# cokwa/bitHTM

Measured on AMD Instinct MI355X. Metric: HTM timesteps/sec (SP + TM, learning on), 65536 cols x 32 cells, higher is better.
Workload: dtype u32 bit-packed / f64 + f32 permanences; 1 GPU; configs[2]: 65536 columns x 32 cells, SP + TM learning on, 1 MI355X; input_dim=1024, column_dim=65536, cell_dim=32, active_columns=1311, patterns=50, pretrain_steps=500, segments=96476, segment_slots=128, hip_graph=True, hip_graph_requested=True, pipelined=True, repetitions=15, streamed_calls=True

## Files before the change

bithtm_amd/_lib.py:

```python

import ctypes as C
import os

HERE = os.path.dirname(os.path.abspath(__file__))
LIB_PATH = os.path.join(HERE, "libbithtm_hip.so")
ABI_VERSION = 4


class HtmConfig(C.Structure):
    _fields_ = [
        ("struct_bytes", C.c_uint32), ("device", C.c_int32),
        ("input_dim", C.c_int32), ("column_dim", C.c_int32), ("cell_dim", C.c_int32),
        ("active_columns", C.c_int32), ("enable_sp", C.c_int32), ("enable_tm", C.c_int32),
        ("sp_permanence_threshold", C.c_double), ("sp_delta_on", C.c_double), ("sp_delta_off", C.c_double),
        ("boost_coefficient", C.c_float), ("duty_momentum", C.c_float), ("duty_increment", C.c_float),
        ("tm_learn_active", C.c_double), ("tm_learn_inactive", C.c_double),
        ("tm_punish_active", C.c_double), ("tm_punish_inactive", C.c_double),
        ("tm_learn_prune", C.c_int32), ("tm_punish_prune", C.c_int32),
        ("tm_permanence_initial", C.c_float), ("tm_permanence_threshold", C.c_float),
        ("segment_activation_threshold", C.c_int32), ("segment_matching_threshold", C.c_int32),
        ("segment_sampling_synapses", C.c_int32),
        ("segment_capacity", C.c_int32), ("segment_capacity_local", C.c_int32), ("segment_slots", C.c_int32),
        ("seed", C.c_uint32), ("shard_rank", C.c_int32), ("shard_world", C.c_int32), ("use_caller_stream", C.c_int32),
        ("stream", C.c_void_p),
    ]


class HtmInfo(C.Structure):
    _fields_ = [
        ("step_index", C.c_int64), ("segments", C.c_int32), ("local_segments", C.c_int32), ("matching_segments", C.c_int32),
        ("winner_cells", C.c_int32), ("active_cells", C.c_int32), ("has_distal_state", C.c_int32),
        ("has_winner_cells", C.c_int32), ("capacity_error", C.c_int32), ("words_per_row", C.c_int32),
        ("new_segment_requests", C.c_int32), ("recycled_segments", C.c_int32), ("appended_segments", C.c_int32),
        ("work_items", C.c_int32), ("select_fallbacks", C.c_int32), ("candidate_exact_steps", C.c_int32), ("hot_select_steps", C.c_int32),
        ("select_zoom_steps", C.c_int32),
    ]


class HtmStepRecord(C.Structure):
    _fields_ = [(name, C.c_int32) for name in (
        "active_columns", "bursting_columns", "predicted_columns_before", "predicted_columns", "active_cells", "winner_cells",
        "segments", "new_segments")]


class HtmRunRecord(C.Structure):
    _fields_ = [("struct_bytes", C.c_uint32), ("records", C.c_void_p), ("active_column", C.c_void_p), ("column_prediction", C.c_void_p)]


F_ACTIVE_COLUMN, F_OVERLAPS, F_BOOSTED, F_DUTY_CYCLE, F_CELL_ACTIVATION, F_CELL_PREDICTION = 1, 2, 3, 4, 5, 6
F_WINNER_WORDS, F_BURSTING, F_WINNER_CELL, F_SEG_CELL, F_SEG_NSYN, F_SEG_PRESYN, F_SEG_PERM = 7, 8, 9, 10, 11, 12, 13
F_SEGCOUNT, F_SEG_POTENTIAL, F_MATCH_SEGMENT, F_MATCH_INFO, F_MATCH_JITTER, F_CELL_MAX_JITTER = 14, 15, 16, 17, 18, 19
F_SEG_GID = 20
PLAN_GRAPH, PLAN_PIPELINED, PLAN_LEAN, PLAN_SCAN_LARGE = 1, 2, 4, 8
SP_OVERLAP, SP_BOOST, SP_SELECT, SP_ACTIVE, SP_LEARN, SP_DUTY, SP_COMMIT = 1, 2, 3, 4, 5, 6, 7

EXPORTS = {
    "htm_abi_version": (C.c_int, []),
    "htm_create": (C.c_int, [C.POINTER(HtmConfig), C.POINTER(C.c_void_p)]),
    "htm_destroy": (None, [C.c_void_p]),
    "htm_last_error": (C.c_char_p, [C.c_void_p]),
    "htm_sp_set_permanence": (C.c_int, [C.c_void_p, C.c_void_p, C.c_int32, C.c_int32]),
    "htm_set_epsilon": (C.c_int, [C.c_void_p, C.c_float]),
    "htm_sp_get_permanence": (C.c_int, [C.c_void_p, C.c_void_p, C.c_int32, C.c_int32]),
    "htm_step": (C.c_int, [C.c_void_p, C.c_void_p, C.c_int32]),
    "htm_sp_step": (C.c_int, [C.c_void_p, C.c_void_p, C.c_int32]),
    "htm_sp_phase": (C.c_int, [C.c_void_p, C.c_int32, C.c_void_p, C.c_int64]),
    "htm_tm_step": (C.c_int, [C.c_void_p, C.c_void_p, C.c_int32, C.c_int32, C.c_int32]),
    "htm_tm_update": (C.c_int, [C.c_void_p, C.c_void_p, C.c_void_p, C.c_void_p, C.c_int32, C.c_void_p]),
    "htm_tm_scan": (C.c_int, [C.c_void_p, C.c_void_p]),
    "htm_run": (C.c_int, [C.c_void_p, C.c_void_p, C.c_int32, C.c_int32, C.c_int32, C.c_int32]),
    "htm_prepare": (C.c_int, [C.c_void_p, C.c_void_p, C.c_int32, C.c_int32, C.c_int32, C.c_int32]),
    "htm_run_recorded": (C.c_int, [C.c_void_p, C.c_void_p, C.c_int32, C.c_int32, C.c_int32, C.c_int32, C.POINTER(HtmRunRecord)]),
    "htm_prepare_recorded": (C.c_int, [C.c_void_p, C.c_void_p, C.c_int32, C.c_int32, C.c_int32, C.c_int32]),
    "htm_reset": (C.c_int, [C.c_void_p]),
    "htm_set_run_resets": (C.c_int, [C.c_void_p, C.c_void_p, C.c_int32]),
    "htm_predicted_input": (C.c_int, [C.c_void_p, C.c_void_p]),
    "htm_set_run_predicted_input": (C.c_int, [C.c_void_p, C.c_void_p]),
    "htm_graph_count": (C.c_int, [C.c_void_p]),
    "htm_run_plan": (C.c_int, [C.c_void_p, C.c_int32, C.c_int32]),
    "htm_bank_upload": (C.c_int, [C.c_void_p, C.c_void_p, C.c_int32, C.POINTER(C.c_void_p)]),
    "htm_shard_record_bytes": (C.c_int64, [C.c_void_p]),
    "htm_shard_begin": (C.c_int, [C.c_void_p, C.c_void_p, C.c_int32, C.c_void_p, C.c_int32, C.c_void_p]),
    "htm_shard_finish": (C.c_int, [C.c_void_p, C.c_void_p, C.c_int32]),
    "htm_shard_unique_id": (C.c_int, [C.c_void_p]),
    "htm_shard_comm_init": (C.c_int, [C.c_void_p, C.c_void_p]),
    "htm_shard_step": (C.c_int, [C.c_void_p, C.c_void_p, C.c_int32, C.c_void_p, C.c_int32]),
    "htm_shard_comm_size": (C.c_int, [C.c_void_p]),
    "htm_shard_graph_ok": (C.c_int, [C.c_void_p]),
    "htm_shard_run": (C.c_int, [C.c_void_p, C.c_void_p, C.c_int32, C.c_int32, C.c_int32, C.c_int32]),
    "htm_shard_group_run": (C.c_int, [C.POINTER(C.c_void_p), C.c_int32, C.POINTER(C.c_void_p), C.c_int32, C.c_int32, C.c_int32, C.c_int32]),
    "htm_rccl_selftest": (C.c_int, [C.c_int32]),
    "htm_keyed_draws": (C.c_int, [C.c_uint32, C.c_int32, C.c_uint32, C.c_void_p, C.c_void_p, C.c_int64, C.c_void_p]),
    "htm_shard_group_step": (C.c_int, [C.POINTER(C.c_void_p), C.c_int32, C.POINTER(C.c_void_p), C.c_int32, C.c_void_p, C.c_int32]),
    "htm_populate": (C.c_int, [C.c_void_p, C.c_int64, C.c_int64, C.c_int32, C.c_int32, C.c_double, C.c_double, C.c_uint32]),
    "htm_sync": (C.c_int, [C.c_void_p]),
    "htm_get_stream": (C.c_int, [C.c_void_p, C.POINTER(C.c_void_p)]),
    "htm_get_info": (C.c_int, [C.c_void_p, C.POINTER(HtmInfo)]),
    "htm_read": (C.c_int64, [C.c_void_p, C.c_int32, C.c_void_p, C.c_int64]),
    "htm_read_rows": (C.c_int64, [C.c_void_p, C.c_int32, C.c_int64, C.c_int64, C.c_void_p, C.c_int64]),
    "htm_import_begin": (C.c_int, [C.c_void_p, C.c_int64]),
    "htm_write": (C.c_int, [C.c_void_p, C.c_int32, C.c_void_p, C.c_int64]),
    "htm_import_commit": (C.c_int, [C.c_void_p, C.c_int32, C.c_int32, C.c_int32, C.c_int32, C.c_int32]),
    "htm_profile": (C.c_int, [C.c_void_p, C.c_int32]),
    "htm_profile_read": (C.c_int, [C.c_void_p, C.c_int32, C.POINTER(C.c_char_p), C.POINTER(C.c_double),
                                   C.POINTER(C.c_int64)]),
# ... 47 lines not shown
```

bithtm_amd/csrc/htm_dev.h:

```cpp
#ifndef BITHTM_HTM_DEV_H
#define BITHTM_HTM_DEV_H

typedef unsigned long long u64;

#define SEL_MAX_PASSES 6
#define SEL_DIGIT 12
#define SEL_BINS 4096
#define HIST_REP 4
#define SEL_COARSE 64
#define COARSE_REP 16
#define COARSE_STRIDE 1024
#define FAN_COUNTERS 16
#define FAN_STRIDE 32
#define HIST0_FINE (HIST_REP * SEL_BINS)
#define HIST0_PAR (HIST0_FINE + COARSE_REP * COARSE_STRIDE)
#define RB 512
#define SCAN_SEGS 64
#define DEAD_CAP 256
#define SHARD_HOT_KEYS 4
#define CAND_CAP 256
#define WIN_LDS 4096
#define MAX_SLOTS 512
#define SYN_CONNECTED 0x80000000u
#define SYN_CELL 0x7FFFFFFF
// ... 24 lines not shown

__host__ __device__ __forceinline__ int sel_shift(int pass) { return pass < 5 ? 52 - SEL_DIGIT * pass : 0; }
__host__ __device__ __forceinline__ int sel_bits(int pass) { return pass < 5 ? SEL_DIGIT : 4; }

struct Counters {
    uint32_t step[2];
    int32_t S;
    int32_t n_win[2];
    int32_t has_winner[2];
    int32_t has_distal;
    uint32_t cm_dense_step;
    int32_t n_active_cells;
    alignas(128) int32_t n_work[2];
    int32_t n_bind[2];
    alignas(128) int32_t n_work_last;
    int32_t sel_fallbacks;
    int32_t cand_exact;
    int32_t hot_selects;
    int32_t sel_zooms;
    uint32_t emit_epoch;
    int32_t n_un;
    int32_t n_recycled, n_new, S_old;
    int32_t L;
    int32_t n_lfree;
    int32_t error;
    u64 sel_prefix[2];
    uint32_t sel_krem[2];
    uint32_t sel_win[2];
    uint32_t sel_win_global;
    u64 sel_pass_prefix[2][SEL_MAX_PASSES + 1];
    uint32_t sel_pass_krem[2][SEL_MAX_PASSES + 1];
};

struct Dev {
    int I, W, W4, Ipad, C, K, k, E, Scap, work_cap, sel_passes, colwords, low_zero, cand_d, cand_pairwise, cand_others, cand_speculate, cand_take_all, cand_zoom, poll_delay;
    int win_offset;
    int cls_rows_max;
    int LK, KP, WPC;
    int world, c0, c1;
    int sel_lo, sel_hi, sel_k;
    int Lcap, n_cand;
    int hot_budget, hot_target;
    int cand_cap;
    double sp_thr, sp_don, sp_doff;
    float coef, mom, dinc;
    double lrn_act, lrn_inact, pun_act, pun_inact;
    int lrn_prune, pun_prune;
    float perm_init, perm_thr;
    float eps;
    int act_thr, match_thr, sample;
    uint32_t seed;
    double *perm;
    uint32_t *mask;
    float *duty;
    int *overlap[2];
    double *boosted[2];
    u64 *key[2];
    uint32_t *hist;
    uint32_t *hist0;
    uint32_t *sel_blk;
    uint32_t *sel_rec;
    int *active_cols[2];
    uint32_t *input_stage;
    uint32_t *act[2];
    uint32_t *pred[2];
    uint32_t *win[2];
    uint32_t *colbits[2];
    int *winners[2];
    uint8_t *bursting;
    int *actw_id;
    uint32_t *winw_idx;
    uint8_t *actcnt;
    uint32_t *act_list;
    uint16_t *col_rank[2];
    uint32_t *unacc_word;
    uint32_t *fan;
    int *unacc_list;
    int *seg_cell;
    int *seg_nsyn;
    int *presyn;
    float *sperm;
    int *segcount;
    uint32_t *cellmax[2];
    uint32_t *match_bits[2];
    uint32_t *seg_info;
    float *seg_jit;
    uint32_t *work;
    int *recyc_cnt;
    int *recyc_cnt2;
    int *recyc_need;
    int *seg_gid;
    int *g2l;
    uint32_t *dead_bits;
    int *lfree;
    int *asg_gid;
    int *cand_cols;
    int *dead_list;
    const uint32_t *punish;
    unsigned char *send;
    Counters *ctr;
    unsigned long long *trace;
    uint32_t trace_until;
};

__device__ __forceinline__ int lane_id() { return threadIdx.x & 63; }
__device__ __forceinline__ u64 lanemask_lt() { return (1ull << lane_id()) - 1ull; }
// ... 156 lines not shown
```

bithtm_amd/csrc/htm_engine.hip:

```cpp

#include <hip/hip_runtime.h>
#include <hip/hip_ext.h>
#include <dlfcn.h>
#include <stdint.h>
#include <stdio.h>
#include <string.h>
#include <algorithm>
#include <climits>
#include <chrono>
#include <map>
#include <mutex>
#include <string>
#include <tuple>
#include <type_traits>
#include <vector>

#include "../../include/bithtm_hip.h"
#include "htm_fexp.h"
#include "htm_rng.h"

#include "htm_dev.h"
#include "htm_sp_kernels.h"
#include "htm_tm_kernels.h"
#include "htm_pipeline.h"
// ... 486 lines not shown

extern "C" int htm_abi_version(void) { return BITHTM_ABI_VERSION; }

extern "C" const char *htm_last_error(const htm_handle *h) { return h ? h->err.c_str() : g_create_error.c_str(); }

extern "C" void htm_destroy(htm_handle *h) {
    if (!h) return;
    {
        std::lock_guard<std::mutex> lock(g_registry_mutex);
        g_registry.erase(std::remove(g_registry.begin(), g_registry.end(), h), g_registry.end());
    }
    hipSetDevice(h->device);
    hipStreamSynchronize(h->stream);
    for (auto &kv : h->graphs) hipGraphExecDestroy(kv.second);
    for (auto &kv : h->shard_graphs) hipGraphExecDestroy(kv.second);
    for (auto &v : h->prof_events)
        for (auto &pr : v) { hipEventDestroy(pr.first); hipEventDestroy(pr.second); }
    for (hipEvent_t e : h->prof_all) hipEventDestroy(e);
    if (h->rccl_comm && g_rccl_destroy) g_rccl_destroy(h->rccl_comm);
    for (void *p : h->allocs) hipFree(p);
    for (void *p : h->weight_allocs) hipFree(p);
    if (h->seg_pinned) hipHostFree(h->seg_pinned);
    if (h->own_stream) hipStreamDestroy(h->stream);
    if (HtmShared *sh = h->shared) {
        bool last;
        {
            std::lock_guard<std::mutex> lock(g_shared_mutex);
            if (sh->parent == h) sh->parent = nullptr;
            last = --sh->refs == 0;
        }
        if (last) {
            for (void *p : sh->allocs) hipFree(p);
            if (sh->own_stream) hipStreamDestroy(sh->stream);
            delete sh;
        }
    }
    delete h;
}

static int fail_create(htm_handle *h, const std::string &msg, int code) {
    g_create_error = msg;
    if (h) { h->err = msg; htm_destroy(h); }
    return code;
}

static int alloc_weights(htm_handle *h) {
    Dev &d = h->d;
    const htm_config *cfg = &h->cfg;
    const size_t C = d.C;
    int rc = 0;
    if (cfg->enable_sp) {
        rc |= dalloc_weights(h, &d.perm, C * d.Ipad);
        rc |= dalloc_weights(h, &d.mask, C * d.W);
    }
    if (cfg->enable_tm) {
        const size_t S = d.Lcap, E = d.E, KP = d.KP;
        rc |= dalloc_weights(h, &d.seg_cell, S);
        rc |= dalloc_weights(h, &d.seg_nsyn, S);
        rc |= dalloc_weights(h, &d.presyn, S * E);
        rc |= dalloc_weights(h, &d.sperm, S * E);
        rc |= dalloc_weights(h, &d.segcount, C * KP);
    }
    return rc;
}

static int alloc_stream_state(htm_handle *h) {
    Dev &d = h->d;
    const htm_config *cfg = &h->cfg;
    const int world = h->world;
    int rc = 0;
    const size_t C = d.C, k = d.k;
    rc |= dalloc(h, &d.ctr, 1);
    rc |= dalloc(h, &d.active_cols[0], k + 8);
    rc |= dalloc(h, &d.active_cols[1], k + 8);
    if (cfg->enable_sp) {
        rc |= dalloc(h, &d.duty, C);
        for (int q = 0; q < 2; ++q) {
            rc |= dalloc(h, &d.overlap[q], C);
            rc |= dalloc(h, &d.boosted[q], C);
            rc |= dalloc(h, &d.key[q], C);
        }
        rc |= dalloc(h, &d.hist, (size_t)2 * SEL_MAX_PASSES * SEL_BINS);
        rc |= dalloc(h, &d.hist0, (size_t)2 * HIST0_PAR);
        rc |= dalloc(h, &d.sel_blk, (C + 255) / 256);
        rc |= dalloc(h, &d.sel_rec, (C + 255) / 256 * 32);
        rc |= dalloc(h, &d.input_stage, (size_t)d.W);
    }
    if (cfg->enable_tm) {
        const size_t S = d.Lcap, G = d.Scap;
        const size_t KP = d.KP, WPC = d.WPC;
        for (int q = 0; q < 2; ++q) {
            rc |= dalloc(h, &d.act[q], C * WPC);
            rc |= dalloc(h, &d.pred[q], C * WPC);
            rc |= dalloc(h, &d.winners[q], k * KP);
        }
        rc |= dalloc(h, &d.win[0], C * WPC);
        rc |= dalloc(h, &d.win[1], C * WPC);
        d.colwords = (int)((C + 63) / 64) * 2;
        const size_t colwords_padded = (size_t)((C + 255) / 256) * 8;
        rc |= dalloc(h, &d.colbits[0], colwords_padded);
        rc |= dalloc(h, &d.colbits[1], colwords_padded);
        rc |= dalloc(h, &d.bursting, k);
        rc |= dalloc(h, &d.actw_id, k * WPC + 8);
        rc |= dalloc(h, &d.winw_idx, k * WPC + 8);
        rc |= dalloc(h, &d.actcnt, k * WPC + 8);
        rc |= dalloc(h, &d.act_list, k * WPC + 16);
// ... 390 lines not shown
    HIPCHK(h, hipStreamSynchronize(h->stream));
    for (auto &kv : h->graphs) hipGraphExecDestroy(kv.second);
    h->graphs.clear();
    h->d.eps = epsilon;
    return HTM_OK;
}

extern "C" int htm_get_stream(htm_handle *h, void **stream) {
    if (!h || !stream) return HTM_ERR_ARGUMENT;
    *stream = (void *)h->stream;
    return HTM_OK;
}

extern "C" int htm_sync(htm_handle *h) {
    if (!h) return HTM_ERR_ARGUMENT;
    if (h) flush_tail(h);
    HIPCHK(h, hipSetDevice(h->device));
    const auto t0 = std::chrono::steady_clock::now();
    for (;;) {
        const hipError_t e = hipStreamQuery(h->stream);
        if (e == hipSuccess) return HTM_OK;
        if (e != hipErrorNotReady) { h->err = std::string("hipStreamQuery: ") + hipGetErrorString(e); return HTM_ERR_HIP; }
        if (std::chrono::steady_clock::now() - t0 > std::chrono::milliseconds(2)) break;
    }
    HIPCHK(h, hipStreamSynchronize(h->stream));
    return HTM_OK;
}

static int check_rows(htm_handle *h, const void *rows, int row_begin, int row_count) {
    if (!h) return HTM_ERR_ARGUMENT;
    if (!h->cfg.enable_sp) { h->err = "handle has no Spatial Pooler"; return HTM_ERR_STATE; }
    if (!rows || row_begin < 0 || row_count < 0 || row_begin + (long long)row_count > h->d.C) {
        h->err = "permanence rows out of range";
        return HTM_ERR_ARGUMENT;
    }
    return 0;
}

extern "C" int htm_sp_set_permanence(htm_handle *h, const double *rows, int32_t row_begin, int32_t row_count) {
    if (h) REFUSE_ON_VIEW(h, "htm_sp_set_permanence");
    if (h) flush_tail(h);
    if (h) weights_touched(h);
    int rc = check_rows(h, rows, row_begin, row_count);
    if (rc) return rc;
    REJECT_WHEN_AHEAD(h);
    if (row_count == 0) return HTM_OK;
    Dev &d = h->d;
    HIPCHK(h, hipSetDevice(h->device));
    HIPCHK(h, hipMemcpy2DAsync(d.perm + (size_t)row_begin * d.Ipad, (size_t)d.Ipad * 8, rows, (size_t)d.I * 8,
                               (size_t)d.I * 8, (size_t)row_count, hipMemcpyHostToDevice, h->stream));
    const long long waves = (long long)row_count * (d.Ipad / 64);
    const int blocks = (int)std::min<long long>((waves + 3) / 4, 8192);
    hipLaunchKernelGGL(k_sp_build_mask, dim3(blocks), dim3(256), 0, h->stream, d, row_begin, row_count);
    HIPCHK(h, hipStreamSynchronize(h->stream));
    return HTM_OK;
}

extern "C" int htm_sp_get_permanence(htm_handle *h, double *rows, int32_t row_begin, int32_t row_count) {
    if (h) flush_tail(h);
    int rc = check_rows(h, rows, row_begin, row_count);
    if (rc) return rc;
    REJECT_WHEN_AHEAD(h);
    if (row_count == 0) return HTM_OK;
    Dev &d = h->d;
    HIPCHK(h, hipSetDevice(h->device));
    HIPCHK(h, hipMemcpy2DAsync(rows, (size_t)d.I * 8, d.perm + (size_t)row_begin * d.Ipad, (size_t)d.Ipad * 8,
                               (size_t)d.I * 8, (size_t)row_count, hipMemcpyDeviceToHost, h->stream));
    HIPCHK(h, hipStreamSynchronize(h->stream));
    return HTM_OK;
}

static int close_open_phases(htm_handle *h) {
    if (!h->phase_open) return 0;
    const int p = (int)(h->step_host & 1);
    if (h->cfg.enable_sp) HIPCHK(h, hipMemsetAsync(h->d.hist0 + (size_t)p * HIST0_PAR, 0, (size_t)HIST0_PAR * 4, h->stream));
    h->phase_open = false;
    h->phase_active = 0;
    return 0;
}

static int stage_input(htm_handle *h, const uint32_t *packed_input) {
    Dev &d = h->d;
    const int words = (d.I + 31) / 32;
    HIPCHK(h, hipMemcpyAsync(d.input_stage, packed_input, (size_t)words * 4, hipMemcpyHostToDevice, h->stream));
    return 0;
}

static decltype(&k_learn_scan_front<1>) const kt_learn_scan_front[4] = {k_learn_scan_front<1>, k_learn_scan_front<2>, k_learn_scan_front<4>, k_learn_scan_front<8>};

extern "C" int htm_step(htm_handle *h, const uint32_t *packed_input, int32_t learning) {
    if (!h || !packed_input) return HTM_ERR_ARGUMENT;
    REJECT_WHEN_AHEAD(h);
    if (!h->cfg.enable_sp || !h->cfg.enable_tm) { h->err = "htm_step needs a handle with SP and TM"; return HTM_ERR_STATE; }
    if (h->world > 1) { h->err = "sharded handle: use htm_shard_begin / htm_shard_finish"; return HTM_ERR_STATE; }
    HIPCHK(h, hipSetDevice(h->device));
    int rc = view_enter(h, learning);
    if (rc) return rc;
    if (learning) weights_touched(h);
    refresh_exchange_mode(h);
    rc = close_open_phases(h);
    if (rc) return rc;
    if (h->d.W > ARG_INPUT_WORDS) {
        flush_tail(h);
        rc = stage_input(h, packed_input);
        if (rc) return rc;
    }
// ... 903 lines not shown
    return 0;
}

extern "C" int htm_get_info(htm_handle *h, htm_info *out) {
    if (!h || !out) return HTM_ERR_ARGUMENT;
    if (h) flush_tail(h);
    Counters c;
    int rc = read_counters(h, &c);
    if (rc) return rc;
    const int q = (int)((h->step_host + 1) & 1);
    const int rows = h->world > 1 ? c.L : c.S;
    out->step_index = h->step_host;
    out->segments = c.S;
    out->local_segments = rows;
    out->matching_segments = 0;
    if (c.has_distal && rows > 0) {
        std::vector<uint32_t> bits(((size_t)rows + 31) / 32);
        HIPCHK(h, hipMemcpy(bits.data(), h->d.match_bits[q], bits.size() * 4, hipMemcpyDeviceToHost));
        for (int i = 0; i < rows; ++i) out->matching_segments += (bits[(size_t)i >> 5] >> (i & 31)) & 1u;
    }
    out->winner_cells = c.n_win[q];
    out->active_cells = c.n_active_cells;
    out->has_distal_state = c.has_distal;
    out->has_winner_cells = h->step_host > 0 ? c.has_winner[q] : 0;
    out->capacity_error = c.error;
    out->words_per_row = h->d.W;
    out->new_segment_requests = c.n_un;
    out->recycled_segments = c.n_un ? c.n_recycled : 0;
    out->appended_segments = c.n_un ? c.n_new : 0;
    out->work_items = c.n_work_last;
    out->select_fallbacks = c.sel_fallbacks;
    out->candidate_exact_steps = c.cand_exact;
    out->hot_select_steps = c.hot_selects;
    out->select_zoom_steps = c.sel_zooms;
    if (c.error) {
        h->err = std::string("capacity exhausted:") + ((c.error & 1) ? " segment pool (segment_capacity)" : "") +
                 ((c.error & 2) ? " synapse slots (segment_slots)" : "") + ((c.error & 4) ? " work list / growth staging" : "") +
                 ((c.error & 8) ? " dead-segment report (DEAD_CAP)" : "") +
                 ((c.error & 16) ? " (internal) block hand-off timed out in k_sp_emit" : "") +
                 ((c.error & 32) ? " (internal) the middle role's wait for the activation blocks timed out in k_act_mid_rows" : "");
        return HTM_ERR_CAPACITY;
    }
    return HTM_OK;
}

static inline int enc_flat(int enc, int K) { return K > 32 ? (enc >> 6) * K + (enc & 63) : (enc >> 5) * K + (enc & 31); }
static inline int flat_enc(int flat, int K) { return (flat / K) * (K > 32 ? 64 : 32) + (flat % K); }

extern "C" int64_t htm_read(htm_handle *h, int32_t field, void *dst, int64_t count) {
    if (!h || !dst) return HTM_ERR_ARGUMENT;
    if (h) flush_tail(h);
    const bool fixed_size = field == HTM_F_ACTIVE_COLUMN || field == HTM_F_OVERLAPS || field == HTM_F_BOOSTED || field == HTM_F_DUTY_CYCLE ||
                            field == HTM_F_CELL_ACTIVATION || field == HTM_F_CELL_PREDICTION || field == HTM_F_WINNER_WORDS ||
                            field == HTM_F_BURSTING || field == HTM_F_SEGCOUNT || field == HTM_F_CELL_MAX_JITTER;
    Counters c;
    memset(&c, 0, sizeof(c));
    int rc = 0;
    if (fixed_size) {
        HIPCHK(h, hipSetDevice(h->device));
        HIPCHK(h, hipStreamSynchronize(h->stream));
    } else {
        rc = read_counters(h, &c);
        if (rc) return rc;
    }
    Dev &d = h->d;
    const int q = (int)((h->step_host + 1) & 1);
    const int qs = h->phase_open ? (int)(h->step_host & 1) : q;
    const bool sp = h->cfg.enable_sp, tm = h->cfg.enable_tm;
    const int64_t C = d.C, K = d.K, S = h->world > 1 ? c.L : c.S, E = d.E, CW = (int64_t)d.C * d.WPC, KP = d.KP;
    auto need = [&](bool ok, int64_t n) -> int64_t {
        if (!ok) { h->err = "htm_read: field not available on this handle"; return HTM_ERR_STATE; }
        if (count < n) { h->err = "htm_read: buffer too small"; return HTM_ERR_ARGUMENT; }
        return n;
    };
    auto copy = [&](const void *src, int64_t n, size_t elem) -> int64_t {
        if (n > 0 && hipMemcpy(dst, src, (size_t)n * elem, hipMemcpyDeviceToHost) != hipSuccess) { h->err = "htm_read: hipMemcpy failed"; return HTM_ERR_HIP; }
        return n;
    };
    int64_t n;
    switch (field) {
        case HTM_F_ACTIVE_COLUMN: if ((n = need(true, d.k)) < 0) return n; return copy(d.active_cols[qs], n, 4);
        case HTM_F_OVERLAPS: REJECT_WHEN_AHEAD(h); if ((n = need(sp, C)) < 0) return n; return copy(d.overlap[qs], n, 4);
        case HTM_F_BOOSTED: REJECT_WHEN_AHEAD(h); if ((n = need(sp, C)) < 0) return n; return copy(d.boosted[qs], n, 8);
        case HTM_F_DUTY_CYCLE: REJECT_WHEN_AHEAD(h); if ((n = need(sp, C)) < 0) return n; return copy(d.duty, n, 4);
        case HTM_F_CELL_ACTIVATION: if ((n = need(tm, CW)) < 0) return n; return copy(d.act[q], n, 4);
        case HTM_F_CELL_PREDICTION: if ((n = need(tm, CW)) < 0) return n; return copy(d.pred[q], n, 4);
        case HTM_F_WINNER_WORDS: if ((n = need(tm, CW)) < 0) return n; return copy(d.win[q], n, 4);
        case HTM_F_BURSTING: if ((n = need(tm, d.k)) < 0) return n; return copy(d.bursting, n, 1);
        case HTM_F_SEG_NSYN: if ((n = need(tm, S)) < 0) return n; return copy(d.seg_nsyn, n, 4);
        case HTM_F_SEG_POTENTIAL:
        case HTM_F_MATCH_SEGMENT:
        case HTM_F_MATCH_INFO:
        case HTM_F_MATCH_JITTER: {
            if (!tm) { h->err = "htm_read: field not available on this handle"; return HTM_ERR_STATE; }
            if (field == HTM_F_SEG_POTENTIAL) {
                if ((n = need(true, S)) < 0) return n;
                if (S == 0) return 0;
                if (!c.has_distal) { memset(dst, 0, (size_t)S * 4); return S; }
                int *tmp = nullptr;
                if (hipMalloc((void **)&tmp, (size_t)S * 4) != hipSuccess) { h->err = "htm_read: hipMalloc failed"; return HTM_ERR_HIP; }
                hipLaunchKernelGGL(k_tm_potentials, dim3((unsigned)std::min<int64_t>((S * 8 + 255) / 256, 8192)), dim3(256), 0, h->stream, d, q, tmp, 0, (int)S);
                const bool ok = hipStreamSynchronize(h->stream) == hipSuccess && hipMemcpy(dst, tmp, (size_t)S * 4, hipMemcpyDeviceToHost) == hipSuccess;
                hipFree(tmp);
                if (!ok) { h->err = "htm_read: potentials kernel failed"; return HTM_ERR_HIP; }
                return S;
            }
            std::vector<uint32_t> bits(((size_t)S + 31) / 32, 0u);
            std::vector<uint32_t> info((size_t)S);
            std::vector<float> jit((size_t)S);
            if (S && c.has_distal && (hipMemcpy(bits.data(), d.match_bits[q], bits.size() * 4, hipMemcpyDeviceToHost) != hipSuccess ||
                                      hipMemcpy(info.data(), d.seg_info, (size_t)S * 4, hipMemcpyDeviceToHost) != hipSuccess ||
                                      hipMemcpy(jit.data(), d.seg_jit, (size_t)S * 4, hipMemcpyDeviceToHost) != hipSuccess)) { h->err = "htm_read: hipMemcpy failed"; return HTM_ERR_HIP; }
            auto is_matching = [&](int64_t i) { return (bits[(size_t)i >> 5] >> (i & 31)) & 1u; };
            int64_t m = 0;
            for (int64_t i = 0; i < S; ++i) m += is_matching(i);
            if ((n = need(true, m)) < 0) return n;
            m = 0;
            for (int64_t i = 0; i < S; ++i) {
                if (!is_matching(i)) continue;
                const uint32_t v = info[(size_t)i];
                if (field == HTM_F_MATCH_SEGMENT) ((int *)dst)[m] = (int)i;
                else if (field == HTM_F_MATCH_INFO) ((uint32_t *)dst)[m] = v & ~0x40000000u;
                else ((float *)dst)[m] = jit[(size_t)i];
                ++m;
            }
            return m;
        }
        case HTM_F_WINNER_CELL:
        case HTM_F_SEG_CELL: {
            const bool w = field == HTM_F_WINNER_CELL;
            if ((n = need(tm, w ? c.n_win[q] : S)) < 0) return n;
            if ((rc = (int)copy(w ? d.winners[q] : d.seg_cell, n, 4)) < 0) return rc;
            int *v = (int *)dst;
            for (int64_t i = 0; i < n; ++i) v[i] = enc_flat(v[i], (int)K);
            return n;
        }
        case HTM_F_SEG_PRESYN:
// ... 814 lines not shown
```

bithtm_amd/csrc/htm_sp_kernels.h:

```cpp
#ifndef BITHTM_HTM_SP_KERNELS_H
#define BITHTM_HTM_SP_KERNELS_H


__global__ __launch_bounds__(256) void k_sp_build_mask(Dev d, int row_begin, int row_count) {
    const int wave = (blockIdx.x * blockDim.x + threadIdx.x) >> 6;
    const int nwaves = (gridDim.x * blockDim.x) >> 6;
    const int lane = lane_id();
    const int chunks = d.Ipad >> 6;
    for (long long t = wave; t < (long long)row_count * chunks; t += nwaves) {
        int row = row_begin + (int)(t / chunks), ch = (int)(t % chunks);
        int i = ch * 64 + lane;
        bool conn = (i < d.I) && (d.perm[(size_t)row * d.Ipad + i] >= d.sp_thr);
        u64 m = __ballot(conn);
        if (lane == 0) *(u64 *)&d.mask[(size_t)row * d.W + ch * 2] = m;
    }
}

#ifdef BITHTM_OVERLAP_STAMPS
#define OV_STAMP(i) do { if (d.trace && wmode && threadIdx.x == 0 && blk < 512) d.trace[(size_t)3 * 8192 + (size_t)blk * 8 + (i)] = wall_clock64(); } while (0)
#else
#define OV_STAMP(i) do { } while (0)
#endif
template <int BS>
__device__ __forceinline__ void role_overlap(const Dev &d, const uint32_t *__restrict__ bank, int n_inputs, int G,
                                             int p, int sp, int step_offset, int blk, int nblk, uint32_t *h, int wmode = 0, int fold = 0) {
    const int gtid = blk * BS + threadIdx.x;
    const int nthreads = nblk * BS;
    uint32_t *ghist = d.hist + sp * SEL_MAX_PASSES * SEL_BINS;
    OV_STAMP(0);
    if (gtid == 0) d.ctr->emit_epoch += 1;
    const uint4 *in4 = (const uint4 *)bank;
    if (n_inputs > 1) in4 = (const uint4 *)(bank + (size_t)((d.ctr->step[p] + (uint32_t)step_offset) % (uint32_t)n_inputs) * d.W);
    const uint4 *mask4 = (const uint4 *)d.mask;
    const int lane = lane_id();
    const int rpw = 64 / G, sub = lane / G, l = lane % G;
    const int wave = gtid >> 6, nwaves = nthreads >> 6;
    constexpr int U = 4;
    const bool spread = G == 8;
    const int first_row0 = d.c0 + wave * rpw * U;
    uint4 m[U];
    float dty_first = 0.f;
    uint32_t cbw_first = 0u;
#pragma unroll
    for (int u = 0; u < U; ++u) {
        const int row = first_row0 + u * rpw + sub;
        m[u] = (row < d.c1 && l < d.W4) ? mask4[(uint32_t)row * (uint32_t)d.W4 + (uint32_t)l] : make_uint4(0, 0, 0, 0);
    }
    if (spread) {
        const int row = first_row0 + (l & 3) * rpw + sub;
        dty_first = (l < U && row < d.c1) ? d.duty[row] : 0.f;
        if (fold) cbw_first = (l < U && row < d.c1) ? d.colbits[p][row >> 5] : 0u;
    }
    for (int i = gtid; i < (d.sel_passes - 1) * SEL_BINS; i += nthreads) ghist[SEL_BINS + i] = 0;
    for (int i = threadIdx.x; i < SEL_BINS; i += BS) h[i] = 0;
    if (gtid == 0) {
        d.ctr->sel_pass_prefix[sp][0] = 0;
        d.ctr->sel_pass_krem[sp][0] = (uint32_t)d.sel_k;
    }
    const uint32_t wbase = wmode ? d.ctr->sel_win[sp] : 0u;
    lds_barrier();
    OV_STAMP(1);
    static_assert(WIN_BINS <= SEL_BINS - SEL_COARSE, "the runs' sums live behind the window's bins in the LDS histogram");
    uint32_t *hc = h + SEL_BINS - SEL_COARSE;
    auto finish_row = [&](bool owner, int row, int cn, float duty, uint32_t cbw) {
        u64 key = 0;
        if (owner && fold) {
            duty = duty * d.mom;
            if ((cbw >> (row & 31)) & 1u) {
                if (fold == 2) owner = false;
                else duty = duty + d.dinc;
            }
            if (owner) d.duty[row] = duty;
        }
        if (owner) {
            d.overlap[sp][row] = cn;
            const float f = htm_exp_f32(d.coef * duty);
            const double bo = (double)f * (double)cn;
            d.boosted[sp][row] = bo;
            key = select_key(bo);
            d.key[sp][row] = key;
        }
        const uint32_t bin = wmode ? win_bin(key, wbase) : (uint32_t)(key >> sel_shift(0));
        if (owner && (!wmode || bin != 0u)) {
            atomicAdd(&h[bin], 1u);
            if (wmode) atomicAdd(&hc[bin >> 6], 1u);
        }
    };
    for (int row0 = first_row0; row0 < d.c1; row0 += nwaves * rpw * U) {
        const bool first = row0 == first_row0;
        int cnt[U];
        float dty = dty_first;
        uint32_t cbw = cbw_first;
#pragma unroll
        for (int u = 0; u < U; ++u) cnt[u] = 0;
        if (!first && spread) {
            const int row = row0 + (l & 3) * rpw + sub;
            dty = (l < U && row < d.c1) ? d.duty[row] : 0.f;
            if (fold) cbw = (l < U && row < d.c1) ? d.colbits[p][row >> 5] : 0u;
        }
        for (int j = l; j < d.W4; j += G) {
            if (!(first && j == l)) {
#pragma unroll
                for (int u = 0; u < U; ++u) {
                    const int row = row0 + u * rpw + sub;
                    m[u] = row < d.c1 ? mask4[(uint32_t)row * (uint32_t)d.W4 + (uint32_t)j] : make_uint4(0, 0, 0, 0);
                }
            }
            const uint4 x = in4[j];
#pragma unroll
            for (int u = 0; u < U; ++u)
                cnt[u] += __popc(m[u].x & x.x) + __popc(m[u].y & x.y) + __popc(m[u].z & x.z) + __popc(m[u].w & x.w);
        }
        OV_STAMP(2);
        if (spread) {
            int mine = 0;
#pragma unroll
            for (int u = 0; u < U; ++u) {
                const int cn = group8_sum_all(cnt[u]);
                if (l == u) mine = cn;
            }
            const int row = row0 + (l & 3) * rpw + sub;
            finish_row(l < U && row < d.c1, row, mine, dty, cbw);
        } else {
#pragma unroll
            for (int u = 0; u < U; ++u) {
                int cn = cnt[u];
                for (int o = G >> 1; o > 0; o >>= 1) cn += __shfl_xor(cn, o);
                const int row = row0 + u * rpw + sub;
                const bool mine = l == 0 && row < d.c1;
                finish_row(mine, row, cn, mine ? d.duty[row] : 0.f, (fold && mine) ? d.colbits[p][row >> 5] : 0u);
            }
        }
    }
    OV_STAMP(3);
    lds_barrier();
    OV_STAMP(4);
    uint32_t *g0 = d.hist0 + (size_t)sp * HIST0_PAR + (size_t)(blk & (HIST_REP - 1)) * SEL_BINS;
    uint32_t *gc = d.hist0 + (size_t)sp * HIST0_PAR + HIST0_FINE + (size_t)(blk & (COARSE_REP - 1)) * COARSE_STRIDE;
    const int n_fine = wmode ? SEL_BINS - SEL_COARSE : SEL_BINS;
    {
        constexpr int PER = SEL_BINS / BS;
// ... 977 lines not shown
                    r_win[pos] = w.winner;
                    r_unacc[pos] = w.unacc;
                }
            }
        }
        for (int i = d.sel_k + b * 256 + tid; i < d.cand_cap; i += nblk * 256) ((u64 *)r_boost)[i] = CAND_PAD;
        if (b == 0) {
            uint32_t *r_dead = r_unacc + d.cand_cap;
            const int n = min(d.dead_list[0], DEAD_CAP);
            if (tid == 0) {
                r_dead[0] = (uint32_t)n;
                uint32_t *r_n = (uint32_t *)(d.send + shard_record_count_offset(d.cand_cap));
                r_n[0] = (uint32_t)d.sel_k;
                r_n[1] = CAND_HOT_NONE;
                if (fused && wmode) d.ctr->cand_exact += 1;
            }
            for (int j = tid; j < n; j += 256) r_dead[1 + j] = (uint32_t)d.dead_list[1 + j];
        }
        return;
    }
    for (int i0 = 0; i0 < n_sel; i0 += tm_groups_per_block(d)) {
        const int i = i0 + tm_group_of(d, tid);
        const bool ok = i < n_sel;
        const int a = ok ? s_col[i] : 0;
        tm_activate_column(d, p, want_winner, ok, a, first_pos + i, d.WPC == 1 ? (u64)(ok ? s_predw[a - cbase] : 0u) : tm_pred_words(d, p, ok, a));
    }
}

__global__ __launch_bounds__(256) void k_sp_emit(Dev d, int p, int want_winner, int fused, int mode, int wmode, int n_emit_blocks) {
    __shared__ EmitShared sh;
    if ((int)blockIdx.x >= n_emit_blocks) {
        const int nb = (int)gridDim.x - n_emit_blocks;
        for (int c = ((int)blockIdx.x - n_emit_blocks) * 256 + (int)threadIdx.x; c < d.C * d.WPC; c += nb * 256) {
            d.act[p][c] = 0;
            d.win[p][c] = 0;
            d.pred[p][c] = 0;
            if (c < d.colwords) d.colbits[p][c] = 0;
        }
        return;
    }
    role_emit(d, p, want_winner, fused, mode, blockIdx.x, n_emit_blocks, &sh, wmode);
}

__global__ __launch_bounds__(256) void k_sp_learn(Dev d, const uint32_t *__restrict__ bank, int n_inputs, int p) {
    const uint32_t *in = bank + (size_t)(d.ctr->step[p] % (uint32_t)n_inputs) * d.W;
    const int row = d.active_cols[p][blockIdx.x];
    double *prow = d.perm + (size_t)row * d.Ipad;
    uint32_t *mrow = d.mask + (size_t)row * d.W;
    for (int i0 = 0; i0 < d.Ipad; i0 += 256) {
        int i = i0 + threadIdx.x;
        bool conn = false;
        if (i < d.I) {
            bool on = (in[i >> 5] >> (i & 31)) & 1u;
            double v = prow[i] + (on ? d.sp_don : d.sp_doff);
            prow[i] = v;
            conn = v >= d.sp_thr;
        }
        u64 m = __ballot(conn);
        if (lane_id() == 0 && i < d.Ipad) *(u64 *)&mrow[i >> 5] = m;
    }
}

__global__ __launch_bounds__(RB) void k_sp_keys(Dev d, int p, int from_overlap) {
    __shared__ uint32_t h[SEL_BINS];
    const int gtid = blockIdx.x * RB + threadIdx.x, nthreads = gridDim.x * RB;
    uint32_t *ghist = d.hist + p * SEL_MAX_PASSES * SEL_BINS;
    if (gtid == 0) {
        d.ctr->emit_epoch += 1;
        d.ctr->sel_pass_prefix[p][0] = 0;
        d.ctr->sel_pass_krem[p][0] = (uint32_t)d.sel_k;
    }
    for (int i = gtid; i < (d.sel_passes - 1) * SEL_BINS; i += nthreads) ghist[SEL_BINS + i] = 0;
    for (int i = threadIdx.x; i < SEL_BINS; i += RB) h[i] = 0;
    __syncthreads();
    for (int c = d.sel_lo + gtid; c < d.sel_hi; c += nthreads) {
        double bo;
        if (from_overlap) {
            const float f = htm_exp_f32(d.coef * d.duty[c]);
            bo = (double)f * (double)d.overlap[p][c];
            d.boosted[p][c] = bo;
        } else {
            bo = d.boosted[p][c];
        }
        const u64 key = select_key(bo);
        d.key[p][c] = key;
        atomicAdd(&h[(uint32_t)(key >> sel_shift(0))], 1u);
    }
    __syncthreads();
    uint32_t *g0 = d.hist0 + (size_t)p * HIST0_PAR + (size_t)(blockIdx.x & (HIST_REP - 1)) * SEL_BINS;
    for (int i = threadIdx.x; i < SEL_BINS; i += RB)
        if (h[i]) atomicAdd(&g0[i], h[i]);
}

__global__ __launch_bounds__(256) void k_sp_list_bits(Dev d, int p, int n, int pass) {
    const int i = blockIdx.x * 256 + threadIdx.x;
    if (pass == 0) { if (i < d.colwords) d.colbits[p][i] = 0; return; }
    if (i < n) { const int c = d.active_cols[p][i]; atomicOr(&d.colbits[p][c >> 5], 1u << (c & 31)); }
}

__global__ __launch_bounds__(256) void k_sp_duty_list(Dev d, int p, int n, int pass) {
    const int i = blockIdx.x * 256 + threadIdx.x;
    if (pass == 0) { if (i < d.C) d.duty[i] = d.duty[i] * d.mom; return; }
    if (i < n) { const int c = d.active_cols[p][i]; d.duty[c] = d.duty[c] + d.dinc; }
}

__global__ void k_sp_commit(Dev d, int p) { d.ctr->step[p ^ 1] = d.ctr->step[p] + 1; }

__global__ __launch_bounds__(RB) void k_shard_overlap(Dev d, const uint32_t *__restrict__ bank, int n_inputs, int G, int p, int wmode, int front) {
    __shared__ uint32_t h[SEL_BINS];
// ... 425 lines not shown
```

bithtm_amd/csrc/htm_tm_kernels.h:

```cpp
#ifndef BITHTM_HTM_TM_KERNELS_H
#define BITHTM_HTM_TM_KERNELS_H


__global__ __launch_bounds__(256) void k_tm_load_active(Dev d, int p, const int *cols, int n) {
    for (int c = blockIdx.x * 256 + threadIdx.x; c < d.C * d.WPC; c += gridDim.x * 256) {
        d.act[p][c] = 0;
        d.pred[p][c] = 0;
        d.win[p][c] = 0;
        if (c < n) d.active_cols[p][c] = cols[c];
        if (c < d.colwords) d.colbits[p][c] = 0;
    }
}

__global__ __launch_bounds__(256) void k_tm_activate(Dev d, int p, int n_active, int want_winner) {
    const int idx = blockIdx.x * tm_groups_per_block(d) + tm_group_of(d, threadIdx.x);
    const bool ok = idx < n_active;
    const int a = ok ? d.active_cols[p][idx] : 0;
    if (ok && (threadIdx.x & (d.KP - 1)) == 0) atomicOr(&d.colbits[p][a >> 5], 1u << (a & 31));
    tm_activate_column(d, p, want_winner, ok, a, idx, tm_pred_words(d, p, ok, a));
}

__global__ __launch_bounds__(256) void k_tm_ext_winners(Dev d, int p, const int *cols, const uint32_t *winw, const uint32_t *unacc, int n, int pass) {
    const int i = blockIdx.x * 256 + threadIdx.x;
    if (pass == 0) { for (int c = i; c < d.C * d.WPC; c += gridDim.x * 256) d.win[p][c] = 0; return; }
// ... 57 lines not shown
        return;
    }
    if (!to_me) return;
    int row = old_row;
    if (row < 0) {
        const int top = atomicSub(&c->n_lfree, 1) - 1;
        if (top >= 0) {
            row = d.lfree[top];
        } else {
            atomicAdd(&c->n_lfree, 1);
            row = atomicAdd(&c->L, 1);
        }
        if (row >= d.Lcap) { atomicOr(&c->error, 1); return; }
        d.seg_gid[row] = gid;
        d.g2l[gid] = row;
    }
    d.seg_cell[row] = cell;
    d.seg_nsyn[row] = (int)SEG_BUSY;
    atomicAdd(&d.segcount[cell], 1);
    const int pos = atomicAdd(&c->n_work[p], 1);
    if (pos < d.work_cap) d.work[pos] = (uint32_t)row; else atomicOr(&c->error, 4);
}

#ifdef BITHTM_ROWS_STAMPS
#define ROW_STAMP(i) do { if (d.trace && t == 0 && ri < 1024) d.trace[(size_t)7 * 8192 + (size_t)ri * 8 + (i)] = wall_clock64(); } while (0)
#else
#define ROW_STAMP(i) do { } while (0)
#endif
template <int TPR, bool OWN = false>
__device__ __forceinline__ void role_sp_row(const Dev &d, int p, const uint32_t *__restrict__ bank, int n_inputs, int ahead, int ri, int t) {
    ROW_STAMP(0);
    const uint32_t step = ahead ? d.ctr->step[p ^ 1] + 1u : d.ctr->step[p];
    const uint32_t *in = bank + (size_t)(step % (uint32_t)n_inputs) * d.W;
    const uint32_t *in_next = bank + (size_t)((step + 1u) % (uint32_t)n_inputs) * d.W;
    const int row = d.active_cols[p][ri];
    if (row < d.c0 || row >= d.c1) return;
    ROW_STAMP(1);
    double *prow = d.perm + (size_t)row * d.Ipad;
    uint32_t *mrow = d.mask + (size_t)row * d.W;
    float duty0 = 0.f;
    uint32_t wbase = 0u;
    if (OWN && t == 0) {
        duty0 = d.duty[row];
        wbase = d.ctr->sel_win[p ^ 1];
    }
    int own_cn = 0;
    for (int i0 = 0; i0 < d.Ipad; i0 += 2 * TPR) {
        const int e0 = i0 + 2 * t;
        bool c0 = false, c1 = false;
        if (e0 < d.Ipad) {
            double2 v = *(double2 *)(prow + e0);
            const uint32_t bits = in[e0 >> 5] >> (e0 & 31);
            const uint32_t nbits = OWN ? in_next[e0 >> 5] >> (e0 & 31) : 0u;
            if (e0 < d.I) { v.x = v.x + ((bits & 1u) ? d.sp_don : d.sp_doff); c0 = v.x >= d.sp_thr; }
            if (e0 + 1 < d.I) { v.y = v.y + ((bits & 2u) ? d.sp_don : d.sp_doff); c1 = v.y >= d.sp_thr; }
            if (OWN) own_cn += (int)(c0 && (nbits & 1u)) + (int)(c1 && (nbits & 2u));
            if (i0 == 0) ROW_STAMP(2); else ROW_STAMP(4);
            {
                typedef unsigned int u32x4 __attribute__((ext_vector_type(4)));
                union { double2 d2; u32x4 u4; } cvt;
                cvt.d2 = v;
                double *dst = prow + e0;
                asm volatile("global_store_dwordx4 %0, %1, off sc0 sc1\n\ts_nop 1" ::"v"(dst), "v"(cvt.u4) : "memory");
            }
        }
        const u64 b0 = __ballot(c0), b1 = __ballot(c1);
        const int base = i0 + 2 * (t & ~63);
        if (lane_id() == 0 && base < d.Ipad) {
            u64 *mw = (u64 *)&mrow[base >> 5];
            const u64 m0 = spread32((uint32_t)b0) | (spread32((uint32_t)b1) << 1);
            const u64 m1 = spread32((uint32_t)(b0 >> 32)) | (spread32((uint32_t)(b1 >> 32)) << 1);
            mw[0] = m0;
            mw[1] = m1;
        }
        if (i0 == 0) ROW_STAMP(3); else ROW_STAMP(5);
    }
    if (OWN) {
        __shared__ int s_own[TPR / 64];
        own_cn = (int)wave_sum((uint32_t)own_cn);
        if (lane_id() == 0) s_own[t >> 6] = own_cn;
        __syncthreads();
        if (t == 0) {
            int cn = 0;
#pragma unroll
            for (int wv = 0; wv < TPR / 64; ++wv) cn += s_own[wv];
            const int sp = p ^ 1;
            float dc = duty0 * d.mom;
            dc = dc + d.dinc;
            d.duty[row] = dc;
            d.overlap[sp][row] = cn;
            const float f = htm_exp_f32(d.coef * dc);
            const double bo = (double)f * (double)cn;
            d.boosted[sp][row] = bo;
            const u64 key = select_key(bo);
            d.key[sp][row] = key;
            const uint32_t bin = win_bin(key, wbase);
            if (bin != 0u) {
                atomicAdd(d.hist0 + (size_t)sp * HIST0_PAR + (size_t)(ri & (HIST_REP - 1)) * SEL_BINS + bin, 1u);
                atomicAdd(d.hist0 + (size_t)sp * HIST0_PAR + HIST0_FINE + (size_t)(ri & (COARSE_REP - 1)) * COARSE_STRIDE + (bin >> 6), 1u);
            }
        }
    }
}

template <typename T>
__device__ __forceinline__ T ld_agent(const T *ptr, int same_launch) {
    return same_launch ? __hip_atomic_load(ptr, __ATOMIC_RELAXED, __HIP_MEMORY_SCOPE_AGENT) : *ptr;
}
// ... 1147 lines not shown
```

include/bithtm_hip.h:

```cpp
#ifndef BITHTM_HIP_H
#define BITHTM_HIP_H

#include <stddef.h>
#include <stdint.h>

#ifdef __cplusplus
extern "C" {
#endif

#define BITHTM_ABI_VERSION 4

typedef struct htm_handle htm_handle;

typedef enum htm_status {
    HTM_OK = 0,
    HTM_ERR_ARGUMENT = -1,
    HTM_ERR_HIP = -2,
    HTM_ERR_CAPACITY = -3,
    HTM_ERR_STATE = -4
} htm_status;

typedef struct htm_config {
    uint32_t struct_bytes;
    int32_t device;
// ... 21 lines not shown
    int32_t segment_matching_threshold;
    int32_t segment_sampling_synapses;
    int32_t segment_capacity;
    int32_t segment_capacity_local;
    int32_t segment_slots;
    uint32_t seed;
    int32_t shard_rank;
    int32_t shard_world;
    int32_t use_caller_stream;
    void *stream;
} htm_config;

typedef struct htm_info {
    int64_t step_index;
    int32_t segments;
    int32_t local_segments;
    int32_t matching_segments;
    int32_t winner_cells;
    int32_t active_cells;
    int32_t has_distal_state;
    int32_t has_winner_cells;
    int32_t capacity_error;
    int32_t words_per_row;
    int32_t new_segment_requests;
    int32_t recycled_segments;
    int32_t appended_segments;
    int32_t work_items;
    int32_t select_fallbacks;
    int32_t candidate_exact_steps;
    int32_t hot_select_steps;
    int32_t select_zoom_steps;
} htm_info;

typedef enum htm_field {
    HTM_F_ACTIVE_COLUMN = 1,
    HTM_F_OVERLAPS = 2,
    HTM_F_BOOSTED = 3,
    HTM_F_DUTY_CYCLE = 4,
    HTM_F_CELL_ACTIVATION = 5,
    HTM_F_CELL_PREDICTION = 6,
    HTM_F_WINNER_WORDS = 7,
    HTM_F_BURSTING = 8,
    HTM_F_WINNER_CELL = 9,
    HTM_F_SEG_CELL = 10,
    HTM_F_SEG_NSYN = 11,
    HTM_F_SEG_PRESYN = 12,
    HTM_F_SEG_PERM = 13,
    HTM_F_SEGCOUNT = 14,
    HTM_F_SEG_POTENTIAL = 15,
    HTM_F_MATCH_SEGMENT = 16,
    HTM_F_MATCH_INFO = 17,
    HTM_F_MATCH_JITTER = 18,
    HTM_F_CELL_MAX_JITTER = 19,
    HTM_F_SEG_GID = 20
} htm_field;

int htm_create(const htm_config *config, htm_handle **out);
void htm_destroy(htm_handle *h);
const char *htm_last_error(const htm_handle *h);
int htm_abi_version(void);

int htm_sp_set_permanence(htm_handle *h, const double *rows, int32_t row_begin, int32_t row_count);

int htm_set_epsilon(htm_handle *h, float epsilon);
int htm_sp_get_permanence(htm_handle *h, double *rows, int32_t row_begin, int32_t row_count);

int htm_step(htm_handle *h, const uint32_t *packed_input, int32_t learning);
int htm_sp_step(htm_handle *h, const uint32_t *packed_input, int32_t learning);
int htm_tm_step(htm_handle *h, const int32_t *active_column, int32_t n, int32_t learning,
                int32_t return_winner_cell);

int htm_tm_update(htm_handle *h, const int32_t *columns, const uint32_t *winner_words, const uint32_t *unaccounted_words,
                  int32_t n, const uint32_t *punish_words);
int htm_tm_scan(htm_handle *h, const uint32_t *active_words);

typedef enum htm_sp_phase_id {
    HTM_SP_OVERLAP = 1,
    HTM_SP_BOOST = 2,
    HTM_SP_SELECT = 3,
    HTM_SP_ACTIVE = 4,
    HTM_SP_LEARN = 5,
    HTM_SP_DUTY = 6,
    HTM_SP_COMMIT = 7
} htm_sp_phase_id;
int htm_sp_phase(htm_handle *h, int32_t phase, const void *data, int64_t count);

int htm_run(htm_handle *h, const uint32_t *device_inputs, int32_t n_inputs, int32_t n_steps,
            int32_t learning, int32_t use_graph);
#define HTM_RUN_GRAPH 1
#define HTM_RUN_NO_PIPELINE 2
#define HTM_RUN_CONTINUE 4

int htm_prepare(htm_handle *h, const uint32_t *device_inputs, int32_t n_inputs, int32_t n_steps,
                int32_t learning, int32_t use_graph);

#define HTM_PLAN_GRAPH 1
#define HTM_PLAN_PIPELINED 2
#define HTM_PLAN_LEAN 4
#define HTM_PLAN_SCAN_LARGE 8
int htm_run_plan(htm_handle *h, int32_t n_steps, int32_t use_graph);

typedef struct htm_step_record {
    int32_t active_columns;
    int32_t bursting_columns;
    int32_t predicted_columns_before;
    int32_t predicted_columns;
    int32_t active_cells;
// ... 86 lines not shown
```

Measured before the change: 42350 timesteps/s.

## Compute SP overlap from an input-major transposed connection mask

Adds a transposed connected-synapse bitmap indexed by input bit, with column words as the minor dimension. It is kept up to date by atomic XOR flips whenever a permanence crosses the threshold during SP learning. With a single device, the overlap kernel walks only the active input bits and gathers column bitmasks for them, instead of scanning every column's full row mask. This aims to cut overlap bandwidth for sparse inputs, but it adds atomic traffic to the learning kernels and an extra mask-build pass.

```diff
diff --git a/bithtm_amd/_lib.py b/bithtm_amd/_lib.py
--- a/bithtm_amd/_lib.py
+++ b/bithtm_amd/_lib.py
@@ -51,6 +51,7 @@
 F_WINNER_WORDS, F_BURSTING, F_WINNER_CELL, F_SEG_CELL, F_SEG_NSYN, F_SEG_PRESYN, F_SEG_PERM = 7, 8, 9, 10, 11, 12, 13
 F_SEGCOUNT, F_SEG_POTENTIAL, F_MATCH_SEGMENT, F_MATCH_INFO, F_MATCH_JITTER, F_CELL_MAX_JITTER = 14, 15, 16, 17, 18, 19
 F_SEG_GID = 20
+F_CONNECTED_BY_INPUT = 21
 PLAN_GRAPH, PLAN_PIPELINED, PLAN_LEAN, PLAN_SCAN_LARGE = 1, 2, 4, 8
 SP_OVERLAP, SP_BOOST, SP_SELECT, SP_ACTIVE, SP_LEARN, SP_DUTY, SP_COMMIT = 1, 2, 3, 4, 5, 6, 7
 
diff --git a/bithtm_amd/csrc/htm_dev.h b/bithtm_amd/csrc/htm_dev.h
--- a/bithtm_amd/csrc/htm_dev.h
+++ b/bithtm_amd/csrc/htm_dev.h
@@ -100,6 +100,8 @@
     uint32_t seed;
     double *perm;
     uint32_t *mask;
+    int cwin;
+    uint32_t *mask_in;
     float *duty;
     int *overlap[2];
     double *boosted[2];
diff --git a/bithtm_amd/csrc/htm_engine.hip b/bithtm_amd/csrc/htm_engine.hip
--- a/bithtm_amd/csrc/htm_engine.hip
+++ b/bithtm_amd/csrc/htm_engine.hip
@@ -562,6 +562,8 @@
     if (cfg->enable_sp) {
         rc |= dalloc_weights(h, &d.perm, C * d.Ipad);
         rc |= dalloc_weights(h, &d.mask, C * d.W);
+        d.cwin = (int)((C + 63) / 64) * 2;
+        rc |= dalloc_weights(h, &d.mask_in, (size_t)d.Ipad * d.cwin);
     }
     if (cfg->enable_tm) {
         const size_t S = d.Lcap, E = d.E, KP = d.KP;
@@ -1058,6 +1060,11 @@
     const long long waves = (long long)row_count * (d.Ipad / 64);
     const int blocks = (int)std::min<long long>((waves + 3) / 4, 8192);
     hipLaunchKernelGGL(k_sp_build_mask, dim3(blocks), dim3(256), 0, h->stream, d, row_begin, row_count);
+    {
+        const int word_begin = row_begin >> 5, word_count = ((row_begin + row_count + 31) >> 5) - word_begin;
+        const long long waves_in = (long long)word_count * (d.Ipad / 64);
+        hipLaunchKernelGGL(k_sp_build_mask_in, dim3((int)std::min<long long>((waves_in + 3) / 4, 8192)), dim3(256), 0, h->stream, d, word_begin, word_count);
+    }
     HIPCHK(h, hipStreamSynchronize(h->stream));
     return HTM_OK;
 }
@@ -2067,7 +2074,8 @@
     if (h) flush_tail(h);
     const bool fixed_size = field == HTM_F_ACTIVE_COLUMN || field == HTM_F_OVERLAPS || field == HTM_F_BOOSTED || field == HTM_F_DUTY_CYCLE ||
                             field == HTM_F_CELL_ACTIVATION || field == HTM_F_CELL_PREDICTION || field == HTM_F_WINNER_WORDS ||
-                            field == HTM_F_BURSTING || field == HTM_F_SEGCOUNT || field == HTM_F_CELL_MAX_JITTER;
+                            field == HTM_F_BURSTING || field == HTM_F_SEGCOUNT || field == HTM_F_CELL_MAX_JITTER ||
+                            field == HTM_F_CONNECTED_BY_INPUT;
     Counters c;
     memset(&c, 0, sizeof(c));
     int rc = 0;
@@ -2098,6 +2106,7 @@
         case HTM_F_OVERLAPS: REJECT_WHEN_AHEAD(h); if ((n = need(sp, C)) < 0) return n; return copy(d.overlap[qs], n, 4);
         case HTM_F_BOOSTED: REJECT_WHEN_AHEAD(h); if ((n = need(sp, C)) < 0) return n; return copy(d.boosted[qs], n, 8);
         case HTM_F_DUTY_CYCLE: REJECT_WHEN_AHEAD(h); if ((n = need(sp, C)) < 0) return n; return copy(d.duty, n, 4);
+        case HTM_F_CONNECTED_BY_INPUT: REJECT_WHEN_AHEAD(h); if ((n = need(sp, (int64_t)d.Ipad * d.cwin)) < 0) return n; return copy(d.mask_in, n, 4);
         case HTM_F_CELL_ACTIVATION: if ((n = need(tm, CW)) < 0) return n; return copy(d.act[q], n, 4);
         case HTM_F_CELL_PREDICTION: if ((n = need(tm, CW)) < 0) return n; return copy(d.pred[q], n, 4);
         case HTM_F_WINNER_WORDS: if ((n = need(tm, CW)) < 0) return n; return copy(d.win[q], n, 4);
diff --git a/bithtm_amd/csrc/htm_sp_kernels.h b/bithtm_amd/csrc/htm_sp_kernels.h
--- a/bithtm_amd/csrc/htm_sp_kernels.h
+++ b/bithtm_amd/csrc/htm_sp_kernels.h
@@ -14,6 +14,27 @@
         u64 m = __ballot(conn);
         if (lane == 0) *(u64 *)&d.mask[(size_t)row * d.W + ch * 2] = m;
     }
+}
+
+__global__ __launch_bounds__(256) void k_sp_build_mask_in(Dev d, int word_begin, int word_count) {
+    const int wave = (blockIdx.x * blockDim.x + threadIdx.x) >> 6;
+    const int nwaves = (gridDim.x * blockDim.x) >> 6;
+    const int lane = lane_id();
+    const int chunks = d.Ipad >> 6;
+    for (long long t = wave; t < (long long)word_count * chunks; t += nwaves) {
+        const int cw = word_begin + (int)(t / chunks), i = (int)(t % chunks) * 64 + lane;
+        uint32_t out = 0u;
+#pragma unroll 8
+        for (int r = 0; r < 32; ++r) {
+            const int row = cw * 32 + r;
+            if (row < d.C && i < d.I && d.perm[(size_t)row * d.Ipad + i] >= d.sp_thr) out |= 1u << r;
+        }
+        d.mask_in[(size_t)i * d.cwin + cw] = out;
+    }
+}
+
+__device__ __forceinline__ void sp_flip(const Dev &d, int i, int row) {
+    atomicXor(&d.mask_in[(size_t)i * d.cwin + (row >> 5)], 1u << (row & 31));
 }
 
 #ifdef BITHTM_OVERLAP_STAMPS
@@ -32,6 +53,7 @@
     const uint4 *in4 = (const uint4 *)bank;
     if (n_inputs > 1) in4 = (const uint4 *)(bank + (size_t)((d.ctr->step[p] + (uint32_t)step_offset) % (uint32_t)n_inputs) * d.W);
     const uint4 *mask4 = (const uint4 *)d.mask;
+    const bool by_input = d.world == 1;
     const int lane = lane_id();
     const int rpw = 64 / G, sub = lane / G, l = lane % G;
     const int wave = gtid >> 6, nwaves = nthreads >> 6;
@@ -44,9 +66,9 @@
 #pragma unroll
     for (int u = 0; u < U; ++u) {
         const int row = first_row0 + u * rpw + sub;
-        m[u] = (row < d.c1 && l < d.W4) ? mask4[(uint32_t)row * (uint32_t)d.W4 + (uint32_t)l] : make_uint4(0, 0, 0, 0);
-    }
-    if (spread) {
+        m[u] = (!by_input && row < d.c1 && l < d.W4) ? mask4[(uint32_t)row * (uint32_t)d.W4 + (uint32_t)l] : make_uint4(0, 0, 0, 0);
+    }
+    if (spread && !by_input) {
         const int row = first_row0 + (l & 3) * rpw + sub;
         dty_first = (l < U && row < d.c1) ? d.duty[row] : 0.f;
         if (fold) cbw_first = (l < U && row < d.c1) ? d.colbits[p][row >> 5] : 0u;
@@ -86,7 +108,46 @@
             if (wmode) atomicAdd(&hc[bin >> 6], 1u);
         }
     };
-    for (int row0 = first_row0; row0 < d.c1; row0 += nwaves * rpw * U) {
+    if (by_input) {
+        const uint32_t *in = (const uint32_t *)in4;
+        const int ncb = (d.c1 - d.c0 + BS - 1) / BS;
+        const int nact = min(nblk, ncb);
+        const int vb = (nact & 7) == 0 ? (blk & 7) * (nact >> 3) + (blk >> 3) : blk;
+        for (int cb = vb; cb < ncb && blk < nact; cb += nact) {
+            const int c = d.c0 + cb * BS + (int)threadIdx.x;
+            const bool mine = c < d.c1;
+            const float dty = mine ? d.duty[c] : 0.f;
+            const uint32_t cbw = (fold && mine) ? d.colbits[p][c >> 5] : 0u;
+            const uint32_t *mw = d.mask_in + ((c - lane) >> 5);
+            const bool wave_in = c - lane < d.c1;
+            int cn = 0, idx = 0, nb = 0;
+            auto drain = [&](int nj) {
+                uint2 w = make_uint2(0u, 0u);
+                if (lane < nj && wave_in) w = *(const uint2 *)(mw + (size_t)idx * (size_t)d.cwin);
+                for (int t = 0; t < nj; ++t) {
+                    const uint32_t lo = wave_read(w.x, t), hi = wave_read(w.y, t);
+                    cn += (int)(((lane < 32 ? lo : hi) >> (lane & 31)) & 1u);
+                }
+            };
+            for (int w0 = 0; w0 < d.W; w0 += 64) {
+                const uint32_t xv = w0 + lane < d.W ? in[w0 + lane] : 0u;
+                const int nw = min(64, d.W - w0);
+                for (int wi = 0; wi < nw; ++wi) {
+                    uint32_t s = wave_read(xv, wi);
+                    while (s) {
+                        const int i = (w0 + wi) * 32 + __builtin_ctz(s);
+                        s &= s - 1u;
+                        if (lane == nb) idx = i;
+                        if (++nb == 64) { drain(64); nb = 0; }
+                    }
+                }
+            }
+            if (nb) drain(nb);
+            OV_STAMP(2);
+            finish_row(mine, c, cn, dty, cbw);
+        }
+    }
+    for (int row0 = first_row0; !by_input && row0 < d.c1; row0 += nwaves * rpw * U) {
         const bool first = row0 == first_row0;
         int cnt[U];
         float dty = dty_first;
@@ -1170,9 +1231,11 @@
         bool conn = false;
         if (i < d.I) {
             bool on = (in[i >> 5] >> (i & 31)) & 1u;
-            double v = prow[i] + (on ? d.sp_don : d.sp_doff);
+            const double v0 = prow[i];
+            const double v = v0 + (on ? d.sp_don : d.sp_doff);
             prow[i] = v;
             conn = v >= d.sp_thr;
+            if (conn != (v0 >= d.sp_thr)) sp_flip(d, i, row);
         }
         u64 m = __ballot(conn);
         if (lane_id() == 0 && i < d.Ipad) *(u64 *)&mrow[i >> 5] = m;
diff --git a/bithtm_amd/csrc/htm_tm_kernels.h b/bithtm_amd/csrc/htm_tm_kernels.h
--- a/bithtm_amd/csrc/htm_tm_kernels.h
+++ b/bithtm_amd/csrc/htm_tm_kernels.h
@@ -133,8 +133,8 @@
             double2 v = *(double2 *)(prow + e0);
             const uint32_t bits = in[e0 >> 5] >> (e0 & 31);
             const uint32_t nbits = OWN ? in_next[e0 >> 5] >> (e0 & 31) : 0u;
-            if (e0 < d.I) { v.x = v.x + ((bits & 1u) ? d.sp_don : d.sp_doff); c0 = v.x >= d.sp_thr; }
-            if (e0 + 1 < d.I) { v.y = v.y + ((bits & 2u) ? d.sp_don : d.sp_doff); c1 = v.y >= d.sp_thr; }
+            if (e0 < d.I) { const bool o = v.x >= d.sp_thr; v.x = v.x + ((bits & 1u) ? d.sp_don : d.sp_doff); c0 = v.x >= d.sp_thr; if (o != c0) sp_flip(d, e0, row); }
+            if (e0 + 1 < d.I) { const bool o = v.y >= d.sp_thr; v.y = v.y + ((bits & 2u) ? d.sp_don : d.sp_doff); c1 = v.y >= d.sp_thr; if (o != c1) sp_flip(d, e0 + 1, row); }
             if (OWN) own_cn += (int)(c0 && (nbits & 1u)) + (int)(c1 && (nbits & 2u));
             if (i0 == 0) ROW_STAMP(2); else ROW_STAMP(4);
             {
diff --git a/include/bithtm_hip.h b/include/bithtm_hip.h
--- a/include/bithtm_hip.h
+++ b/include/bithtm_hip.h
@@ -97,7 +97,8 @@
     HTM_F_MATCH_INFO = 17,
     HTM_F_MATCH_JITTER = 18,
     HTM_F_CELL_MAX_JITTER = 19,
-    HTM_F_SEG_GID = 20
+    HTM_F_SEG_GID = 20,
+    HTM_F_CONNECTED_BY_INPUT = 21
 } htm_field;
 
 int htm_create(const htm_config *config, htm_handle **out);
```

Result: slower. 41490 timesteps/s, median of 2 (-2.0%).
